# DrQuestion/monica

Measured on AMD Instinct MI355X. Metric: reads/sec classified, higher is better.
Workload: dtype u32/u64 integer; int16 pairs in the alignment kernels (int32 / int8 in the long-call and literal ones); float32 islands: overlap ratio, MAPQ

## Files before the change

monica_amd/csrc/engine.hip:

```cpp
#include <hip/hip_runtime.h>
#include <algorithm>
#include <cmath>
#include <cstdio>
#include <cstring>
#include <cstdlib>
#include <new>
#include <vector>

#include "device.h"
#include <atomic>
#include <thread>

#include "scan.h"

namespace mnc {

void launch_pack(const Batch &B, hipStream_t st);
void launch_sketch(const Batch &B, hipStream_t st);
void launch_partition(const Batch &B, hipStream_t st);
int partition_prepare();
void launch_probe(const Batch &B, hipStream_t st);
void launch_collect(const Batch &B, hipStream_t st);
void launch_expand_sort(const Batch &B, const uint32_t *lists, const ClassSpans &spans, int NM, hipStream_t st);
int expand_sort_prepare(int max_nm);
void launch_backtrack(const Batch &B, const uint32_t *read_list, uint32_t n_list, hipStream_t st);
void launch_bin_reads(const Batch &B, const ChainClasses &C, uint32_t *cls_count, uint32_t *cls_list, hipStream_t st);
void launch_chain_dp_ring(const Batch &B, const uint32_t *lists, const ClassSpans &spans, int stress, hipStream_t st);
void launch_chain_tail(const Batch &B, const uint32_t *lists, const ClassSpans &spans, int NM, hipStream_t st);
size_t chain_tail_lds_bytes(int NM);
int chain_tail_prepare(size_t max_lds);

static const ChainClasses CHAIN_CLASSES = { 22, { 64, 128, 192, 256, 320, 384, 448, 512, 576, 640, 768, 896, 1024, 1280, 1536, 1792, 2048, 2560,
                                                  3072, 4096, 6144, 8192 } };
void launch_regions(const Batch &B, void *regx, uint64_t *k64a, uint64_t *k64b, mnc_hit_t *gated, hipStream_t st);
void launch_regions_post(const Batch &B, mnc_reg_t *work, void *regx, uint64_t *k64a, int32_t *tmp, mnc_hit_t *gated, hipStream_t st);
void launch_dp_gather(const Batch &B, hipStream_t st);
int dp_gather_long_prepare(int lds_anchors);
void launch_dp_gather_long(const Batch &B, const uint32_t *lists, const ClassSpans &spans, int lds_anchors, hipStream_t st);
void launch_dp_round(const Batch &B, int first, hipStream_t st);
void launch_dp_round_end(const Batch &B, hipStream_t st);
int dp_plan_prepare();
void launch_dp_plan(const Batch &B, const int32_t *work_list, unsigned max_work, int wave_form, int state_max, long long p_max, int cig_max,
                    long long big_state, long long big_p, long long big_cig, long long huge_state, long long huge_p, long long huge_cig, hipStream_t st);
size_t dp_align_ws_bytes(long long state_max, long long p_max, long long cig_max);
int dp_align_prepare(int lds_bytes);
int dp_stitch_prepare();
size_t dp_inv_ws_words(int max_gap);
void launch_dp_inv(const Batch &B, const int32_t *work_list, int32_t *next_list, int32_t *ws, int n_wg, hipStream_t st);
size_t dp_stitch_pool_slack(int n_wg);
void launch_dp_align(const Batch &B, uint8_t *ws, int n_wg, long long state_max, long long p_max, long long cig_max,
                     int lds_state, int lds_p, int lds_cig, int big_pass, hipStream_t st, int forms = 3);
void launch_dp_stitch(const Batch &B, const int32_t *work_list, int32_t *next_list, int max_read_len, int n_wg, hipStream_t st);
bool dp_align_long_packed(const Batch &B);
void launch_dp_align_long(const Batch &B, uint8_t *ws_huge, int n_huge, long long st_huge, long long p_huge, long long cig_huge,
                          uint8_t *ws_big, int n_big, long long st_big, long long p_big, long long cig_big,
                          uint8_t *ws_small, int n_small, long long st_small, long long p_small, long long cig_small, hipStream_t st);
size_t dp_fill_p_slot();
size_t dp_fillp_slot();
// ... 48 lines not shown
__global__ __launch_bounds__(PB_N_MAX) void mnc_hist_offsets(const uint32_t *hist_tm, uint32_t n_tiles, uint32_t n_chunks,
                                                             const int64_t *chunk_off_bm, int64_t *q_off)
{
	const uint32_t c = blockIdx.x, b = threadIdx.x, PB_N = blockDim.x;
	const uint32_t t0 = c * HC_TILES, t1 = min(n_tiles, t0 + HC_TILES);
	int64_t run = chunk_off_bm[(size_t)b * n_chunks + c];
	for (uint32_t t = t0; t < t1; ++t) {
		q_off[(size_t)t * PB_N + b] = run;
		run += hist_tm[(size_t)t * PB_N + b];
	}
	if (c == 0 && b == 0) q_off[(size_t)n_tiles * PB_N] = chunk_off_bm[(size_t)PB_N * n_chunks];
}

struct MailItem { const void *src; uint32_t dst_word, n_words; };
constexpr int MAIL_MAX = 8;
struct MailList { MailItem it[MAIL_MAX]; int n; };
__global__ __launch_bounds__(64) void mnc_mail(MailList L, uint32_t *host_box)
{
	for (int k = 0; k < L.n; ++k) {
		const uint32_t *s = static_cast<const uint32_t*>(L.it[k].src);
		for (uint32_t i = threadIdx.x; i < L.it[k].n_words; i += 64) host_box[L.it[k].dst_word + i] = s[i];
	}
	__threadfence_system();
}

struct Buf {
	void *p = nullptr;
	size_t cap = 0;
	int ensure(size_t bytes)
	{
		if (bytes <= cap) return MNC_OK;
		if (p) { (void)hipFree(p); p = nullptr; cap = 0; }
		size_t want = bytes + bytes / 8 + 256;
		hipError_t e = hipMalloc(&p, want);
		if (e != hipSuccess) { p = nullptr; set_error("hipMalloc(%zu) failed: %s", want, hipGetErrorString(e)); return MNC_ERR_NOMEM; }
		cap = want;
		return MNC_OK;
	}
	void release() { if (p) (void)hipFree(p); p = nullptr; cap = 0; }
	template <class T> T *as() const { return reinterpret_cast<T*>(p); }
};

struct SharedWs {
	std::mutex mu;
	int refs = 0;
	Buf fill_p, fill_cig, extp_p, extp_cig, ext_p, lfill_p, lext_p, dp_ws, dp_ws_mid, dp_ws_big, dp_ws_bigfb, dp_ws_huge;
// ... 230 lines not shown
	Buf pf_bases_buf, pf_offsets_buf;
	hipStream_t copy_stream = nullptr;
	hipEvent_t ev_prefetch = nullptr;
	std::mutex pf_mu;
	bool pf_valid = false;
	const uint8_t *pf_bases = nullptr;
	const int64_t *pf_offsets = nullptr;
	uint32_t pf_n = 0;
	int64_t pf_total = 0;
	Buf packed, mz, hits, hist_tm, q_off, qrec, bhits, bhit_cnt;
	size_t q_cap_override = 0;
	Buf ambig, skip, mz_cnt, hit_cnt, rep_len, an_cnt, an_off, n_chain, n_reg, scan_sums, hit_off, best_mlen, hist_sums, hist_offs;
	Buf a, f, p, v, t, u;
	Buf chains_tmp, regs, regx, k64a, k64b, tmp_i32, gated, hits_csr;
	Buf stats, cls_count, cls_list;
	int contract = MNC_CONTRACT_DP;
	Buf ca, ca_cnt, chain_dst, regdp, segs, cig_seg, cig_reg, dp_ctr, work_a, work_b, big_list, huge_list, reg_cnt, regs2;
	SharedWs *ws = nullptr;
	Buf fill1, fill2, fill3, fill_mid, fill_fb, plan_long, extp, mid_list, lfill, lext, bigfb, ext1, ext2, ext3, ext4, gen_list;
	size_t seg_cap_override = 0, cig_cap_override = 0;
	uint32_t *mailbox = nullptr;
	int last_redos = 0;
	long long prev_wide_calls = 0;
	int slot_pad = 2;
	Buf inv_ws;
	int cur_max_read_len = 0;
	int long_reads = 0;
	bool cur_wide = false;
	bool have_merged = false;
	std::vector<int64_t> merged_off;
	std::vector<mnc_hit_t> merged_hits;
	int64_t merged_ctr[24]{};
	Buf ex_off, ex_alns, ex_coff, ex_csoff, ex_mdoff, ex_sums, ex_cigar, ex_cs, ex_md;
	bool ex_valid = false;
	int64_t ex_n_reads = 0, ex_n_aln = 0, ex_n_cig = 0, ex_n_cs = 0, ex_n_md = 0;
	hipEvent_t ev_ex[2]{};
	bool ev_ex_used = false;
	int debug = 0;
	Batch B{};
	bool have_batch = false;
	int64_t last_total_anchors = 0, last_total_hits = -1;
	std::vector<int64_t> h_offsets;
	bool profiling = false;
	hipEvent_t ev[MNC_N_STAGES][2]{};
	bool ev_used[MNC_N_STAGES]{};
	double ms[MNC_N_STAGES]{};
// ... 128 lines not shown
{
	if (n <= e->logf_n) return MNC_OK;
	std::vector<float> lg, lga;
	try { lg.resize((size_t)n), lga.resize((size_t)n); } catch (const std::bad_alloc &) { set_error("out of host memory (MAPQ look-ups)"); return MNC_ERR_NOMEM; }
	for (int i = 0; i < n; ++i) lg[i] = logf((float)i), lga[i] = logf((float)i / e->idx->par.a);
	int rc = e->logf_lut.ensure((size_t)n * 4);
	if (!rc) rc = e->logf_a_lut.ensure((size_t)n * 4);
	if (rc) { e->logf_n = 0; return rc; }
	HIP_TRY(hipMemcpy(e->logf_lut.p, lg.data(), (size_t)n * 4, hipMemcpyHostToDevice));
	HIP_TRY(hipMemcpy(e->logf_a_lut.p, lga.data(), (size_t)n * 4, hipMemcpyHostToDevice));
	e->logf_n = n;
	return MNC_OK;
}

extern "C" int mnc_engine_create(mnc_index *idx, int device, mnc_engine **out)
{
	if (!idx || !out) return MNC_ERR_ARG;
	*out = nullptr;
	if (int rc = check_device(device)) return rc;
	if (idx->par.bw >= GAP_LUT) { set_error("bw too large for the gap look-up"); return MNC_ERR_UNSUPPORTED; }
	mnc_engine *e = new (std::nothrow) mnc_engine;
	if (!e) return MNC_ERR_NOMEM;
	e->idx = idx, e->device = device;
	e->ws = shared_ws(device, +1);
	int rc = index_upload(idx, device, &e->didx);
	if (rc) { mnc_engine_destroy(e); return rc; }
	hipError_t he = hipSetDevice(device);
	int least = 0, greatest = 0;
	if (he == hipSuccess) {
		if (hipDeviceGetStreamPriorityRange(&least, &greatest) != hipSuccess) least = greatest = 0;
		he = hipStreamCreateWithPriority(&e->stream, hipStreamNonBlocking, greatest);
	}
	for (int k = 0; k < mnc_engine::N_SIDE && he == hipSuccess; ++k) {
		he = k < 3 ? hipStreamCreateWithFlags(&e->side[k], hipStreamNonBlocking) : hipStreamCreateWithPriority(&e->side[k], hipStreamNonBlocking, greatest);
		if (he == hipSuccess) he = hipEventCreateWithFlags(&e->ev_join[k], hipEventDisableTiming);
	}
	if (he == hipSuccess) he = hipEventCreateWithFlags(&e->ev_fork, hipEventDisableTiming);
	if (he == hipSuccess) he = hipEventCreateWithFlags(&e->ev_lfill, hipEventDisableTiming);
	if (he == hipSuccess) he = hipStreamCreateWithPriority(&e->copy_stream, hipStreamNonBlocking, least);
	if (he == hipSuccess) he = hipEventCreateWithFlags(&e->ev_prefetch, hipEventDisableTiming);
	if (he == hipSuccess) he = hipHostMalloc((void**)&e->mailbox, 1024, hipHostMallocDefault);
	if (he != hipSuccess) { set_error("stream creation failed: %s", hipGetErrorString(he)); mnc_engine_destroy(e); return MNC_ERR_HIP; }
	for (int s = 0; s < MNC_N_STAGES; ++s) for (int k = 0; k < 2; ++k) (void)hipEventCreate(&e->ev[s][k]);
	std::vector<int32_t> gap(GAP_LUT);
	const float avg_span = (float)idx->k;
	for (int dd = 0; dd < GAP_LUT; ++dd) {
// ... 197 lines not shown
	mark(MNC_STAGE_DP_FILL_T2, 1), mark(MNC_STAGE_DP_FILL_T3, 0);
	launch_dp_fill(B, 128, B.fill_list3, 22, 23, B.fill_fb, 12, B.fill_fb, 12, e->ws->fill_p.as<uint8_t>(), e->ws->fill_cig.as<uint32_t>(), DP_WG_FILL, s0);
	if (!serial && !packed_long && small_batch) long_passes(s0);
	mark(MNC_STAGE_DP_FILL_T3, 1), mark(MNC_STAGE_DP_LFILL, 0);
	if (serial) launch_dp_lfill(B, B.lfill_list, 31, 61, B.fill_fb, 12, e->ws->lfill_p.as<uint8_t>(), DP_WG_LFILL, s0);
	mark(MNC_STAGE_DP_LFILL, 1), mark(MNC_STAGE_DP_EXT, 0);
	for (int i = 7; i >= 0; --i)
		launch_dp_extp(B, 32 << (i >> 1), i & 1, B.extp_list + (int64_t)i * B.seg_cap, 32 + i, 40 + i, e->ws->extp_p.as<uint8_t>(), e->ws->extp_cig.as<uint32_t>(), DP_WG_EXT, s1);
	launch_dp_ext(B, 32, B.ext_list1, 16, 18, B.fill_fb, 12, e->ws->ext_p.as<uint8_t>(), DP_WG_EXT, s1);
	launch_dp_ext(B, 64, B.ext_list2, 17, 19, B.fill_fb, 12, e->ws->ext_p.as<uint8_t>(), DP_WG_EXT, s1);
	launch_dp_ext(B, 128, B.ext_list3, 24, 26, B.fill_fb, 12, e->ws->ext_p.as<uint8_t>(), DP_WG_EXT / 2, s1);
	launch_dp_ext(B, 256, B.ext_list4, 25, 27, B.fill_fb, 12, e->ws->ext_p.as<uint8_t>(), DP_WG_EXT / 4, s1);
	mark(MNC_STAGE_DP_EXT, 1);
	if (serial) {
		launch_dp_lext(B, B.lext_list, 62, 63, B.fill_fb, 12, e->ws->lext_p.as<uint8_t>(), DP_WG_LEXT, s0);
		long_passes(s0);
	}
	launch_dp_align(B, e->ws->dp_ws.as<uint8_t>(), 2 * DP_WG_SMALL, DP_STATE_SMALL, DP_P_SMALL, DP_CIG_SMALL, DP_LDS0_STATE, DP_LDS0_P, DP_LDS0_CIG, 0, s2);
}
static void align_rest(const Batch &B, mnc_engine *e, hipStream_t st)
{
	launch_dp_align(B, e->ws->dp_ws.as<uint8_t>(), DP_WG_SMALL, DP_STATE_SMALL, DP_P_SMALL, DP_CIG_SMALL, DP_LDS_BYTES, 0, 0, 2, st);
	launch_dp_align(B, e->ws->dp_ws_big.as<uint8_t>(), (dp_align_long_packed(B) && !(e->debug & 0x10000)) ? 64 : DP_WG_BIG, DP_STATE_BIG, DP_P_BIG, DP_CIG_BIG, DP_LDS_BYTES, 0, 0, 4, st);
}

static int classify_once(mnc_engine *e, const uint8_t *d_bases, const int64_t *d_offsets,
                         uint32_t n_reads, int64_t total_bases, int min_mapq,
                         int32_t *d_assign, mnc_hit_t *d_best, int32_t *d_nhits, int64_t *d_counts, int *overflowed)
{
	hipStream_t st = e->stream;
	const mnc_index *idx = e->idx;
	*overflowed = 0;
	const size_t nr = (size_t)n_reads, nb = (size_t)total_bases;
	const int pb_bits = e->didx->pb_bits;
	const size_t PB_N = (size_t)1 << pb_bits, PS_TILES = (size_t)(e->cur_wide ? PS_TILES_MIN / 2 : PS_TILES_MIN);
	const size_t n_tiles = (nr + PT_READS - 1) / PT_READS, n_super = (n_tiles + PS_TILES - 1) / PS_TILES;
	size_t q_cap = nb / 3 + 4096;
	if (e->q_cap_override > q_cap) q_cap = e->q_cap_override < nb + 4096 ? e->q_cap_override : nb + 4096;

	int rc = MNC_OK;
#define ENS(buf, bytes) do { if (!rc) rc = e->buf.ensure(bytes); } while (0)
	ENS(packed, (nb / 16 + 4) * 4);
	ENS(mz, (nb + 1) * sizeof(uint2));
	ENS(hits, (nb + 1) * sizeof(HitRec));
	ENS(ambig, (nr + 1) * 4);
	ENS(skip, (nr + 1) * 4);
// ... 43 lines not shown
	B.gap_lut = e->gap_lut.as<int32_t>(), B.logf_lut = e->logf_lut.as<float>(), B.logf_a_lut = e->logf_a_lut.as<float>(), B.logf_n = e->logf_n;
	B.debug_route = (e->debug >> 17 & 15) | ((e->debug >> 22 & 1) << 4) | ((e->debug >> 5 & 1) << 5)
	              | ((e->debug >> 6 & 1) << 6) | ((e->debug >> 7 & 1) << 7)
	              | ((e->debug >> 3 & 1) << 8) | ((e->debug & 1) << 9)
	              | (((unsigned)e->debug >> 31 & 1) << 10);
	B.fill_pred = (e->debug >> 8 & 0xff) ? (e->debug >> 8 & 0xff) : 32;
	B.fill_pred_mid = (e->debug >> 24 & 0x7f) ? (e->debug >> 24 & 0x7f) : 34;
	B.fill_pred_auto = !(e->debug >> 8 & 0xff) && !(e->debug >> 24 & 0x7f) && P.a == 2 && P.b == 4 && P.q == 4 && P.e == 2 &&
	                   P.q2 == 24 && P.e2 == 1 && !getenv("MNC_FILL_PRED_FIXED");
	B.contract = e->contract, B.seq4 = e->didx->seq4, B.seq_off = e->didx->seq_off;
	B.sc_a = P.a, B.sc_b = P.b, B.gap_q = P.q, B.gap_e = P.e, B.gap_q2 = P.q2, B.gap_e2 = P.e2, B.sc_ambi = P.sc_ambi;
	B.zdrop = P.zdrop, B.zdrop_inv = P.zdrop_inv, B.end_bonus = P.end_bonus, B.min_dp_max = P.min_dp_max, B.min_ksw_len = P.min_ksw_len;
	B.max_sw_mat = P.max_sw_mat;
	B.packed = e->packed.as<uint32_t>(), B.ambig = e->ambig.as<uint32_t>(), B.skip = e->skip.as<uint32_t>(), B.mz = e->mz.as<uint2>(), B.hits = e->hits.as<HitRec>();
	B.mz_cnt = e->mz_cnt.as<int32_t>(), B.hit_cnt = e->hit_cnt.as<int32_t>(), B.rep_len = e->rep_len.as<int32_t>();
	B.an_cnt = e->an_cnt.as<int64_t>(), B.an_off = e->an_off.as<int64_t>(), B.n_chain = e->n_chain.as<int32_t>(), B.n_reg = e->n_reg.as<int32_t>(), B.best_mlen = e->best_mlen.as<int32_t>();
	B.n_tiles = (uint32_t)n_tiles, B.n_super = (uint32_t)n_super;
	B.hist_tm = e->hist_tm.as<uint32_t>(), B.q_off = e->q_off.as<int64_t>(), B.qrec = e->qrec.as<uint64_t>();
	B.q_cap = (int64_t)q_cap, B.bhits = e->bhits.as<HitRec>(), B.bhit_cnt = e->bhit_cnt.as<uint32_t>();
	B.overflow = reinterpret_cast<uint32_t*>(e->stats.as<int64_t>() + 8);
	B.assign = d_assign, B.best = d_best, B.nhits = d_nhits ? d_nhits : e->out_nhits.as<int32_t>(), B.counts = d_counts;
	B.stats = e->stats.as<int64_t>();

	HIP_TRY(hipMemsetAsync(B.ambig, 0, (nr + 1) * 4, st));
	HIP_TRY(hipMemsetAsync(B.skip, 0, (nr + 1) * 4, st));
	HIP_TRY(hipMemsetAsync(B.packed + nb / 16, 0, 16, st));
	HIP_TRY(hipMemsetAsync(B.overflow, 0, 8, st));

	{ StageTimer t(e, MNC_STAGE_PACK);   launch_pack(B, st); }
	{ StageTimer t(e, MNC_STAGE_SKETCH); launch_sketch(B, st); }
	{
		StageTimer t(e, MNC_STAGE_PARTITION);
		{
			const uint32_t n_chunks = (uint32_t)((n_tiles + HC_TILES - 1) / HC_TILES);
			uint32_t *sums_bm = e->hist_sums.as<uint32_t>();
			int64_t *off_bm = e->hist_offs.as<int64_t>();
			hipLaunchKernelGGL(mnc_hist_chunk_sums, dim3(n_chunks), dim3((unsigned)PB_N), 0, st, B.hist_tm, (uint32_t)n_tiles, n_chunks, sums_bm);
			exclusive_scan(ScanInPlain<uint32_t>{sums_bm}, (int64_t)n_chunks * PB_N, off_bm, e->scan_sums.as<int64_t>(), st);
			hipLaunchKernelGGL(mnc_hist_offsets, dim3(n_chunks), dim3((unsigned)PB_N), 0, st, B.hist_tm, (uint32_t)n_tiles, n_chunks, off_bm, B.q_off);
		}
		launch_partition(B, st);
	}
	{ StageTimer t(e, MNC_STAGE_PROBE);   launch_probe(B, st); }
	{ StageTimer t(e, MNC_STAGE_COLLECT); launch_collect(B, st); }
	HIP_TRY(hipGetLastError());
	int64_t total_anchors = 0, total_q = 0;
	uint32_t cls_count[MAX_CHAIN_CLASSES + 1] = {0}, overflow = 0;
	{
		StageTimer t(e, MNC_STAGE_SORT);
		exclusive_scan(ScanInPlain<int64_t>{B.an_cnt}, (int64_t)n_reads, B.an_off, e->scan_sums.as<int64_t>(), st);
		HIP_TRY(hipMemsetAsync(e->cls_count.p, 0, (MAX_CHAIN_CLASSES + 1) * 4, st));
		launch_bin_reads(B, CHAIN_CLASSES, e->cls_count.as<uint32_t>(), e->cls_list.as<uint32_t>(), st);
		MailList ml;
		ml.n = 4;
		ml.it[0] = { B.an_off + n_reads, 0, 2 }, ml.it[1] = { B.q_off + n_tiles * PB_N, 2, 2 };
		ml.it[2] = { e->cls_count.p, 4, (uint32_t)(MAX_CHAIN_CLASSES + 1) }, ml.it[3] = { B.overflow, 4 + MAX_CHAIN_CLASSES + 1, 1 };
		hipLaunchKernelGGL(mnc_mail, dim3(1), dim3(64), 0, st, ml, e->mailbox);
		HIP_TRY(hipStreamSynchronize(st));
		memcpy(&total_anchors, e->mailbox, 8), memcpy(&total_q, e->mailbox + 2, 8);
		memcpy(cls_count, e->mailbox + 4, (MAX_CHAIN_CLASSES + 1) * 4);
		overflow = e->mailbox[4 + MAX_CHAIN_CLASSES + 1];
	}
	if (overflow || total_q > (int64_t)q_cap) {
		e->q_cap_override = (size_t)total_q + (size_t)total_q / 8 + 4096;
		*overflowed = 1;
		return MNC_OK;
	}
	if (total_anchors < 0 || total_anchors >= (1LL << 31) * 16) { set_error("anchor count %lld out of range", (long long)total_anchors); return MNC_ERR_UNSUPPORTED; }
	e->last_total_anchors = total_anchors;
	const size_t na = (size_t)total_anchors + 4, ns = (size_t)total_anchors / 3 + 4, nsr = ns + nr * (size_t)e->slot_pad;
	ENS(a, na * sizeof(Anchor));
	ENS(f, na * 4); ENS(p, na * 4); ENS(v, na * 4); ENS(t, na * 4);
	ENS(u, na * 8);
	ENS(chains_tmp, ns * sizeof(ChainRec));
// ... 2 lines not shown
	if (rc) return rc;
#undef ENS
	B.an_cap = (int64_t)na;
	B.slot_pad = e->slot_pad;
	B.a = e->a.as<Anchor>(), B.chains_tmp = e->chains_tmp.as<ChainRec>();
	B.f = e->f.as<int32_t>(), B.p = e->p.as<int32_t>(), B.v = e->v.as<int32_t>(), B.t = e->t.as<int32_t>(), B.u = e->u.as<uint64_t>();
	B.regs = e->regs.as<mnc_reg_t>(), B.tmp_i32 = e->tmp_i32.as<int32_t>();

	auto fork = [&]() -> int {
		HIP_TRY(hipEventRecord(e->ev_fork, st));
		for (int k = 0; k < mnc_engine::N_SIDE; ++k) HIP_TRY(hipStreamWaitEvent(e->side[k], e->ev_fork, 0));
		return MNC_OK;
	};
	auto join = [&]() -> int {
		for (int k = 0; k < mnc_engine::N_SIDE; ++k) {
			HIP_TRY(hipEventRecord(e->ev_join[k], e->side[k]));
			HIP_TRY(hipStreamWaitEvent(st, e->ev_join[k], 0));
		}
		return MNC_OK;
	};
	{
		StageTimer t(e, MNC_STAGE_SORT2);
		const uint32_t *lists = e->cls_list.as<uint32_t>();
		if (int rc = fork()) return rc;
		constexpr int SORT_MERGE = 512;
		int first_big = 0;
		while (first_big < CHAIN_CLASSES.n && CHAIN_CLASSES.nm[first_big] <= SORT_MERGE) ++first_big;
		int k = 0;
		if (first_big > 0) {
			ClassSpans sp;
			sp.n = first_big, sp.stride = (uint32_t)n_reads, sp.start[0] = 0;
			for (int c = 0; c < first_big; ++c) sp.start[c + 1] = sp.start[c] + cls_count[c];
			if (sp.start[sp.n]) launch_expand_sort(B, lists, sp, CHAIN_CLASSES.nm[first_big - 1], e->side[k++ % mnc_engine::N_SIDE]);
		}
		for (int c = first_big; c <= CHAIN_CLASSES.n; ++c) {
			if (cls_count[c] == 0) continue;
			ClassSpans sp;
			sp.n = 1, sp.stride = 0, sp.start[0] = 0, sp.start[1] = cls_count[c];
			launch_expand_sort(B, lists + (size_t)c * n_reads, sp, c < CHAIN_CLASSES.n ? CHAIN_CLASSES.nm[c] : 0,
			                   e->side[k++ % mnc_engine::N_SIDE]);
		}
		if (int rc = join()) return rc;
	}
	{
		StageTimer t(e, MNC_STAGE_CHAIN);
		const uint32_t *lists = e->cls_list.as<uint32_t>();
		ClassSpans spans;
		spans.n = CHAIN_CLASSES.n + 1, spans.stride = (uint32_t)n_reads, spans.start[0] = 0;
		for (int c = 0; c <= CHAIN_CLASSES.n; ++c) spans.start[c + 1] = spans.start[c] + cls_count[c];
		launch_chain_dp_ring(B, lists, spans, (e->debug & 2) != 0, st);
	}
	{
		StageTimer t(e, MNC_STAGE_BACKTRACK);
		const uint32_t *lists = e->cls_list.as<uint32_t>();
		if (int rc = fork()) return rc;
		int k = 0;
		constexpr int merge_to = 384;
		int first_big = 0;
		while (first_big < CHAIN_CLASSES.n && CHAIN_CLASSES.nm[first_big] <= merge_to) ++first_big;
		if (first_big > 0) {
			ClassSpans sp;
			sp.n = first_big, sp.stride = (uint32_t)n_reads, sp.start[0] = 0;
			for (int c = 0; c < first_big; ++c) sp.start[c + 1] = sp.start[c] + cls_count[c];
			if (sp.start[sp.n]) launch_chain_tail(B, lists, sp, CHAIN_CLASSES.nm[first_big - 1], e->side[k++ % mnc_engine::N_SIDE]);
		}
		for (int c = first_big; c < CHAIN_CLASSES.n; ++c) {
			if (cls_count[c] == 0) continue;
			ClassSpans sp;
			sp.n = 1, sp.stride = 0, sp.start[0] = 0, sp.start[1] = cls_count[c];
			launch_chain_tail(B, lists + (size_t)c * n_reads, sp, CHAIN_CLASSES.nm[c], e->side[k++ % mnc_engine::N_SIDE]);
		}
		launch_backtrack(B, lists + (size_t)CHAIN_CLASSES.n * n_reads, cls_count[CHAIN_CLASSES.n], e->side[k % mnc_engine::N_SIDE]);
		if (int rc = join()) return rc;
	}
	if (e->contract == MNC_CONTRACT_DP) {
		size_t seg_cap = na / 6 + 4096, cig_cap = nb / 2 + (1u << 20);
		if (e->seg_cap_override > seg_cap) seg_cap = e->seg_cap_override;
		if (e->cig_cap_override > cig_cap) cig_cap = e->cig_cap_override;
		int rc2 = MNC_OK;
#define ENS2(buf, bytes) do { if (!rc2) rc2 = e->buf.ensure(bytes); } while (0)
#define ENSW(buf, bytes) do { if (!rc2) rc2 = e->ws->buf.ensure(bytes); } while (0)
		std::unique_lock<std::mutex> ws_hold(e->ws->mu);
		ENS2(ca, na * sizeof(Anchor)); ENS2(ca_cnt, (nr + 1) * 4); ENS2(chain_dst, ns * 4); ENS2(regdp, nsr * sizeof(RegDP));
		ENS2(inv_ws, dp_inv_ws_words(B.max_gap) * 4 * DP_WG_INV);
		const size_t cig_reg_cap = cig_cap + dp_stitch_pool_slack(DP_WG_STITCH);
		ENS2(segs, seg_cap * sizeof(Seg)); ENS2(cig_seg, cig_cap * 4); ENS2(cig_reg, cig_reg_cap * 4);
		ENS2(work_a, nsr * 4); ENS2(work_b, nsr * 4); ENS2(big_list, seg_cap * 4); ENS2(reg_cnt, (nr + 1) * 4); ENS2(regs2, nsr * sizeof(mnc_reg_t));
		const size_t ws_small = dp_align_ws_bytes(DP_STATE_SMALL, DP_P_SMALL, DP_CIG_SMALL), ws_big = dp_align_ws_bytes(DP_STATE_BIG, DP_P_BIG, DP_CIG_BIG), ws_huge = dp_align_ws_bytes(DP_STATE_HUGE, DP_P_HUGE, DP_CIG_HUGE);
		ENSW(dp_ws, ws_small * DP_WG_SMALL * 2); ENSW(dp_ws_big, ws_big * DP_WG_BIG); ENSW(dp_ws_bigfb, ws_big * DP_WG_BIGFB); ENSW(dp_ws_huge, ws_huge * DP_WG_HUGE); ENS2(huge_list, seg_cap * 4); ENSW(dp_ws_mid, ws_small * DP_WG_MID); ENS2(mid_list, seg_cap * 4); ENS2(lfill, seg_cap * 4); ENSW(lfill_p, dp_lfill_p_slot() * DP_WG_LFILL); ENS2(lext, seg_cap * 4); ENS2(bigfb, seg_cap * 4); ENSW(lext_p, dp_lext_p_slot() * DP_WG_LEXT);
		ENS2(plan_long, (nr * 4 + 1024) * 4);
		ENS2(fill1, seg_cap * 4); ENS2(fill2, seg_cap * 4); ENS2(fill3, seg_cap * 4); ENS2(fill_mid, seg_cap * 4); ENS2(fill_fb, seg_cap * 4); ENSW(fill_p, dp_fillp_slot() * DP_WG_FILL); ENSW(fill_cig, dp_fillp_cig_slot() * DP_WG_FILL); ENS2(extp, seg_cap * 4 * 8); ENSW(extp_p, dp_extp_slot() * DP_WG_EXT); ENSW(extp_cig, dp_extp_cig_slot() * DP_WG_EXT); ENS2(ext1, seg_cap * 4); ENS2(ext2, seg_cap * 4); ENS2(ext3, seg_cap * 4); ENS2(ext4, seg_cap * 4); ENS2(gen_list, seg_cap * 4); ENSW(ext_p, dp_fill_p_slot() * DP_WG_EXT);
#undef ENS2
		if (rc2) return rc2;
		B.ca = e->ca.as<Anchor>(), B.ca_cnt = e->ca_cnt.as<int32_t>(), B.chain_dst = e->chain_dst.as<int32_t>(), B.regdp = e->regdp.as<RegDP>();
		B.segs = e->segs.as<Seg>(), B.seg_cap = (int64_t)seg_cap, B.cig_seg = e->cig_seg.as<uint32_t>(), B.cig_reg = e->cig_reg.as<uint32_t>();
		B.cig_seg_cap = (int64_t)cig_cap, B.cig_reg_cap = (int64_t)cig_reg_cap, B.dp_ctr = e->dp_ctr.as<unsigned long long>();
		B.big_list = e->big_list.as<int32_t>(), B.huge_list = e->huge_list.as<int32_t>(), B.reg_cnt = e->reg_cnt.as<int32_t>();
		B.plan_long_list = e->plan_long.as<int32_t>(), B.plan_long_cap = (long long)(nr * 4 + 1024);
		B.fill_list1 = e->fill1.as<int32_t>(), B.fill_list2 = e->fill2.as<int32_t>(), B.fill_list3 = e->fill3.as<int32_t>(), B.fill_list_mid = e->fill_mid.as<int32_t>(), B.fill_fb = e->fill_fb.as<int32_t>();
		B.ext_list1 = e->ext1.as<int32_t>(), B.ext_list2 = e->ext2.as<int32_t>(), B.ext_list3 = e->ext3.as<int32_t>(), B.ext_list4 = e->ext4.as<int32_t>(), B.gen_list = e->gen_list.as<int32_t>(), B.extp_list = e->extp.as<int32_t>(), B.mid_list = e->mid_list.as<int32_t>(), B.lfill_list = e->lfill.as<int32_t>(), B.lext_list = e->lext.as<int32_t>(), B.bigfb_list = e->bigfb.as<int32_t>();
		B.lds0_state = DP_LDS0_STATE, B.lds0_p = DP_LDS0_P, B.lds0_cig = DP_LDS0_CIG;
		int32_t *lists[2] = { e->work_a.as<int32_t>(), e->work_b.as<int32_t>() };
		B.next_list = lists[0];
		HIP_TRY(hipMemsetAsync(e->dp_ctr.p, 0, 64 * 8, st));
		{ StageTimer t(e, MNC_STAGE_REGIONS);   launch_regions(B, e->regx.p, e->k64a.as<uint64_t>(), e->k64b.as<uint64_t>(), e->gated.as<mnc_hit_t>(), st); }
		{
			StageTimer t(e, MNC_STAGE_DP_PLAN);
			launch_dp_gather(B, st);
			int c0 = 0;
			while (c0 < CHAIN_CLASSES.n && CHAIN_CLASSES.nm[c0] <= 1024) ++c0;
			ClassSpans sp;
			sp.n = CHAIN_CLASSES.n + 1 - c0, sp.stride = (uint32_t)n_reads, sp.start[0] = 0;
			for (int c = c0; c <= CHAIN_CLASSES.n; ++c) sp.start[c - c0 + 1] = sp.start[c - c0] + cls_count[c];
			launch_dp_gather_long(B, e->cls_list.as<uint32_t>() + (size_t)c0 * n_reads, sp, CHAIN_CLASSES.nm[CHAIN_CLASSES.n - 1], st);
		}
		unsigned max_work = (unsigned)nsr;
		const int long_reads = (e->debug & 0x10) ? 2 : (e->debug & 0x800000) ? 0 : n_reads <= 4096 ? 2
		                     : (e->cur_max_read_len <= 0 || e->cur_max_read_len > 6144) ? 1 : 0;
		for (int round = 0;; ++round) {
			const int32_t *work = lists[round & 1];
			int32_t *next = lists[(round + 1) & 1];
			B.next_list = next;
			launch_dp_round(B, round == 0, st);
			if (round == 0) {
				{ StageTimer t(e, MNC_STAGE_DP_PLAN);   launch_dp_plan(B, work, max_work, long_reads, (int)DP_STATE_SMALL, DP_P_SMALL, (int)DP_CIG_SMALL, DP_STATE_BIG, DP_P_BIG, DP_CIG_BIG, DP_STATE_HUGE, DP_P_HUGE, DP_CIG_HUGE, st); }
				{
					StageTimer t(e, MNC_STAGE_DP_FILL);
					if (int rcf = fork()) return rcf;
					if (e->debug & 0x10000) align_round(B, e, e->side[0], e->side[0], e->side[0], e->side[0], e->side[0]);
					else align_round(B, e, e->side[0], e->side[1], st, e->side[2], e->side[3]);
					if (int rcj = join()) return rcj;
				}
				{
					StageTimer t(e, MNC_STAGE_DP_ALIGN);
					align_rest(B, e, st);
				}
				{ StageTimer t(e, MNC_STAGE_DP_STITCH); launch_dp_stitch(B, work, next, (e->debug & 0x200000) ? 0 : e->cur_max_read_len > 0 ? e->cur_max_read_len : 8192, DP_WG_STITCH, st); }
			} else {
				launch_dp_plan(B, work, max_work, long_reads, (int)DP_STATE_SMALL, DP_P_SMALL, (int)DP_CIG_SMALL, DP_STATE_BIG, DP_P_BIG, DP_CIG_BIG, DP_STATE_HUGE, DP_P_HUGE, DP_CIG_HUGE, st);
				if (int rcf = fork()) return rcf;
				if (e->debug & 0x10000) align_round(B, e, e->side[0], e->side[0], e->side[0], e->side[0], e->side[0]);
				else align_round(B, e, e->side[0], e->side[1], st, e->side[2], e->side[3]);
				if (int rcj = join()) return rcj;
				align_rest(B, e, st);
				launch_dp_stitch(B, work, next, (e->debug & 0x200000) ? 0 : e->cur_max_read_len > 0 ? e->cur_max_read_len : 8192, DP_WG_STITCH, st);
				launch_dp_inv(B, work, next, e->inv_ws.as<int32_t>(), (int)std::min<unsigned>(DP_WG_INV, max_work), st);
			}
			launch_dp_round_end(B, st);
			unsigned long long ctr[6] = {0};
			{
				MailList ml;
				ml.n = 3;
				ml.it[0] = { e->dp_ctr.p, 0, 12 };
				ml.it[1] = { e->dp_ctr.as<unsigned long long>() + 6, 12, 2 }, ml.it[2] = { e->dp_ctr.as<unsigned long long>() + 58, 14, 2 };
				hipLaunchKernelGGL(mnc_mail, dim3(1), dim3(64), 0, st, ml, e->mailbox);
				HIP_TRY(hipStreamSynchronize(st));
				memcpy(ctr, e->mailbox, sizeof(ctr));
				if (round == 0 && n_reads >= 4096) {
					unsigned long long big = 0, huge = 0;
					memcpy(&big, e->mailbox + 12, 8), memcpy(&huge, e->mailbox + 14, 8);
					e->prev_wide_calls = (long long)(big + huge);
				}
			}
			if (ctr[4] != 0) {
				if (ctr[4] >= 9) { set_error("a gap between two seeds is too large for the alignment workspace"); return MNC_ERR_UNSUPPORTED; }
				if (ctr[4] == 5) {
					e->slot_pad = e->slot_pad * 4;
					*overflowed = 2;
					return MNC_OK;
				}
				e->seg_cap_override = na + 2 * ns + 1024;
				e->cig_cap_override = cig_cap * 4;
				*overflowed = 2;
				return MNC_OK;
			}
			if (ctr[5] == 0) break;
			if (round > 256) { set_error("base-level alignment does not settle"); return MNC_ERR_HIP; }
			max_work = (unsigned)ctr[5];
		}
		{ StageTimer t(e, MNC_STAGE_DP_POST); launch_regions_post(B, e->regs2.as<mnc_reg_t>(), e->regx.p, e->k64a.as<uint64_t>(), e->tmp_i32.as<int32_t>(), e->gated.as<mnc_hit_t>(), st); }
	} else {
		StageTimer t(e, MNC_STAGE_REGIONS);
		launch_regions(B, e->regx.p, e->k64a.as<uint64_t>(), e->k64b.as<uint64_t>(), e->gated.as<mnc_hit_t>(), st);
	}
	HIP_TRY(hipGetLastError());
	e->have_batch = true;
	return MNC_OK;
}

extern "C" int mnc_classify_device(mnc_engine *e, const uint8_t *d_bases, const int64_t *d_offsets,
                                   uint32_t n_reads, int64_t total_bases, int max_read_len, int min_mapq,
                                   int32_t *d_assign, mnc_hit_t *d_best, int32_t *d_nhits, int64_t *d_counts)
{
	if (!e || !d_offsets || !d_assign || (total_bases > 0 && !d_bases) || total_bases < 0) return MNC_ERR_ARG;
	if (((uintptr_t)d_bases & 15u) != 0) { set_error("d_bases must be 16-byte aligned"); return MNC_ERR_ARG; }
	const bool wide = e->long_reads && max_read_len >= (1 << QPOS_BITS);
	if (max_read_len < 0 || (wide ? max_read_len > MNC_MAX_READ_LEN_WIDE : max_read_len >= (1 << QPOS_BITS))) {
		set_error(e->long_reads ? "reads beyond 2^24 - 1 bases are not supported" : "reads of 2^20 bases or more are not supported (mnc_engine_set_long_reads)");
		return MNC_ERR_UNSUPPORTED;
	}
	if (n_reads > (1u << 20)) { set_error("at most 2^20 reads per batch (query records hold a 20-bit read ordinal)"); return MNC_ERR_UNSUPPORTED; }
	if (wide && n_reads > (uint32_t)WIDE_MAX_READS) { set_error("at most 2^16 reads in a call with reads of 2^20 bases or more (wide query records hold a 16-bit read ordinal)"); return MNC_ERR_UNSUPPORTED; }
	if (total_bases >= (1LL << 40)) return MNC_ERR_UNSUPPORTED;
// ... 545 lines not shown
```

monica_amd/csrc/k_post.hip:

```cpp
#include "device.h"

namespace mnc {

__device__ __forceinline__ uint64_t mix64(uint64_t key)
{
	key = ~key + (key << 21);
	key = key ^ key >> 24;
	key = (key + (key << 3)) + (key << 8);
	key = key ^ key >> 14;
	key = (key + (key << 2)) + (key << 4);
	key = key ^ key >> 28;
	key = key + (key << 31);
	return key;
}

__device__ __forceinline__ uint32_t wang32(uint32_t key)
{
	key += ~(key << 15);
	key ^=  (key >> 10);
	key +=  (key << 3);
	key ^=  (key >> 6);
	key += ~(key << 11);
	key ^=  (key >> 16);
	return key;
// ... 393 lines not shown
			for (int i = 0; i < n_regs; ++i) total += rg[i].cnt;
			B.ca_cnt[rd] = total;
			if (n_regs > 0) {
				const unsigned long long w0 = atomicAdd(&B.dp_ctr[5], (unsigned long long)n_regs);
				for (int i = 0; i < n_regs; ++i) {
					RegDP d;
					memset(&d, 0, sizeof(d));
					d.read = (int32_t)rd, d.order = i << 8, d.state = 1;
					B.regdp[slot + i] = d;
					B.next_list[w0 + i] = (int32_t)(slot + i);
				}
			}
		}
	} else if (dp) B.ca_cnt[rd] = 0;
	if (dp) { B.reg_cnt[rd] = n_regs; return; }
	B.n_reg[rd] = n_regs;
	B.assign[rd] = assign;
	if (B.best) B.best[rd] = best;
	B.nhits[rd] = nhits;
	B.best_mlen[rd] = best.mlen;
}

__global__ __launch_bounds__(64) void mnc_regions_post(Batch B, mnc_reg_t *work_all, RegX *regx_all, uint64_t *k64a_all,
                                                       int32_t *tmp_all, mnc_hit_t *gated_all)
{
	const uint32_t rd = blockIdx.x * blockDim.x + threadIdx.x;
	if (rd >= B.n_reads) return;
	int32_t assign = MNC_UNMAPPED, nhits = 0;
	mnc_hit_t best;
	best.rid = best.mapq = best.nm = best.mlen = 0;
	const int n0 = B.reg_cnt[rd];
	int n_regs = 0;
	if (n0 > 0) {
		const int64_t slot = reg_slot(B, rd);
		mnc_reg_t *src = B.regs + slot, *r = work_all + slot;
		RegX *ex = regx_all + slot;
		uint64_t *ka = k64a_all + slot;
		int32_t *w = tmp_all + slot * 4, *tmp = w + n0;
		mnc_hit_t *gated = gated_all + slot;
		for (int i = 0; i < n0; ++i) w[i] = i;
		for (int i = 1; i < n0; ++i) {
			const int c = w[i], oc = B.regdp[slot + c].order;
			int j = i - 1;
			while (j >= 0 && B.regdp[slot + w[j]].order > oc) { w[j + 1] = w[j]; --j; }
			w[j + 1] = c;
		}
		int k = 0;
		for (int i = 0; i < n0; ++i) {
			const mnc_reg_t x = src[w[i]];
			bool flt = !(x.flags & REG_INV) && x.cnt < B.min_cnt;
// ... 23 lines not shown
			}
			for (int i = 0; i < n_regs; ++i) src[i] = r[tmp[i]], B.regdp[slot + i].cig_off = (int64_t)ex[tmp[i]].x0;
			for (int i = 0; i < n_regs; ++i) { r[i] = src[i]; RegX e; e.x0 = (uint64_t)B.regdp[slot + i].cig_off, e.y0 = 0, e.x1 = (uint64_t)(uint32_t)src[i].n_cigar, e.y1 = 0; ex[i] = e; }
		}
		set_parent(B, n_regs, r, ka, w);
		n_regs = select_sub(B, n_regs, r, ex, tmp);
		set_mapq(B, rd, n_regs, r);
		gate_and_decide(B, n_regs, r, gated, assign, best, nhits);
		for (int i = 0; i < n_regs; ++i) src[i] = r[i], B.regdp[slot + i].cig_off = (int64_t)ex[i].x0, B.regdp[slot + i].n_cigar = r[i].n_cigar;
	}
	if (B.skip[rd]) {
		assign = MNC_SKIPPED, nhits = 0;
		memset(&best, 0, sizeof(best));
	}
	B.n_reg[rd] = n_regs;
	B.assign[rd] = assign;
	if (B.best) B.best[rd] = best;
	B.nhits[rd] = nhits;
	B.best_mlen[rd] = best.mlen;
}

constexpr int CT_THREADS = 256, CT_READS = 4096, CT_LDS_BINS = 3 * 1024;

__global__ __launch_bounds__(CT_THREADS) void mnc_count_taxa(Batch B)
{
	__shared__ unsigned long long s_bins[CT_LDS_BINS];
	const int n_bins = B.n_genomes * 3;
	const bool in_lds = n_bins <= CT_LDS_BINS;
	if (in_lds) {
		for (int k = threadIdx.x; k < n_bins; k += CT_THREADS) s_bins[k] = 0;
		__syncthreads();
	}
	unsigned long long *bins = in_lds ? s_bins : (unsigned long long*)B.counts;
	const uint32_t lo = blockIdx.x * CT_READS;
	const uint32_t hi = min(B.n_reads, lo + CT_READS);
	for (uint32_t rd = lo + threadIdx.x; rd < hi; rd += CT_THREADS) {
		const int a = B.assign[rd];
		if (a < 0) continue;
		const int g = B.contig_genome[a];
		atomicAdd(&bins[g * 3 + 0], 1ULL);
		atomicAdd(&bins[g * 3 + 1], (unsigned long long)(B.offsets[rd + 1] - B.offsets[rd]));
		atomicAdd(&bins[g * 3 + 2], (unsigned long long)B.best_mlen[rd]);
	}
	if (in_lds) {
		__syncthreads();
		for (int k = threadIdx.x; k < n_bins; k += CT_THREADS)
			if (s_bins[k]) atomicAdd((unsigned long long*)&B.counts[k], s_bins[k]);
	}
}

__global__ __launch_bounds__(256) void mnc_gather_hits(Batch B, const mnc_hit_t *gated_all,
                                                       const int64_t *hit_off, mnc_hit_t *out)
{
	const uint32_t rd = blockIdx.x * blockDim.x + threadIdx.x;
	if (rd >= B.n_reads) return;
	const int n = B.nhits[rd];
	if (n == 0) return;
	const mnc_hit_t *src = gated_all + reg_slot(B, rd);
	mnc_hit_t *dst = out + hit_off[rd];
	for (int i = 0; i < n; ++i) dst[i] = src[i];
}

void launch_regions(const Batch &B, void *regx, uint64_t *k64a, uint64_t *k64b, mnc_hit_t *gated, hipStream_t st)
{
	if (B.n_reads == 0) return;
	hipLaunchKernelGGL(mnc_regions_decide, dim3((B.n_reads + 63) / 64), dim3(64), 0, st, B,
	                   reinterpret_cast<RegX*>(regx), k64a, k64b, gated);
	if (B.counts && B.contract != MNC_CONTRACT_DP)
		hipLaunchKernelGGL(mnc_count_taxa, dim3((B.n_reads + CT_READS - 1) / CT_READS), dim3(CT_THREADS), 0, st, B);
}

void launch_regions_post(const Batch &B, mnc_reg_t *work, void *regx, uint64_t *k64a, int32_t *tmp, mnc_hit_t *gated, hipStream_t st)
{
	if (B.n_reads == 0) return;
	hipLaunchKernelGGL(mnc_regions_post, dim3((B.n_reads + 63) / 64), dim3(64), 0, st, B, work,
	                   reinterpret_cast<RegX*>(regx), k64a, tmp, gated);
	if (B.counts) hipLaunchKernelGGL(mnc_count_taxa, dim3((B.n_reads + CT_READS - 1) / CT_READS), dim3(CT_THREADS), 0, st, B);
}

void launch_gather_hits(const Batch &B, const mnc_hit_t *gated, const int64_t *hit_off, mnc_hit_t *out, hipStream_t st)
{
	if (B.n_reads == 0) return;
	hipLaunchKernelGGL(mnc_gather_hits, dim3((B.n_reads + 255) / 256), dim3(256), 0, st, B, gated, hit_off, out);
}

}
```

Measured before the change: 2.875 million.

## Fuse batch clears into one kernel, gate side-stream fork, speculatively queue post stage

Replaces the per-batch hipMemsetAsync calls (ambig, skip, packed tail, overflow, class counts, DP counters) with a single clearing kernel. It forks onto side streams for the sort and backtrack stages only when the work outside the largest class exceeds a threshold, and otherwise launches everything on the main stream. It also queues the regions-post and count-taxa kernels before the first host sync, gated on device counters so they exit early if more DP rounds are needed. The aim is fewer API calls, fewer cross-stream event waits and less idle time after the host sync, at the cost of more complex control flow and possibly lost overlap for small batches. The old behaviour is kept behind the MNC_HOST_WAITS environment variable.

```diff
diff --git a/monica_amd/csrc/engine.hip b/monica_amd/csrc/engine.hip
--- a/monica_amd/csrc/engine.hip
+++ b/monica_amd/csrc/engine.hip
@@ -33,7 +33,7 @@
 static const ChainClasses CHAIN_CLASSES = { 22, { 64, 128, 192, 256, 320, 384, 448, 512, 576, 640, 768, 896, 1024, 1280, 1536, 1792, 2048, 2560,
                                                   3072, 4096, 6144, 8192 } };
 void launch_regions(const Batch &B, void *regx, uint64_t *k64a, uint64_t *k64b, mnc_hit_t *gated, hipStream_t st);
-void launch_regions_post(const Batch &B, mnc_reg_t *work, void *regx, uint64_t *k64a, int32_t *tmp, mnc_hit_t *gated, hipStream_t st);
+void launch_regions_post(const Batch &B, mnc_reg_t *work, void *regx, uint64_t *k64a, int32_t *tmp, mnc_hit_t *gated, const unsigned long long *gate, hipStream_t st);
 void launch_dp_gather(const Batch &B, hipStream_t st);
 int dp_gather_long_prepare(int lds_anchors);
 void launch_dp_gather_long(const Batch &B, const uint32_t *lists, const ClassSpans &spans, int lds_anchors, hipStream_t st);
@@ -128,6 +128,20 @@
 		for (uint32_t i = threadIdx.x; i < L.it[k].n_words; i += 64) host_box[L.it[k].dst_word + i] = s[i];
 	}
 	__threadfence_system();
+}
+
+static_assert(MAX_CHAIN_CLASSES + 1 <= 256, "mnc_clear_batch clears the class counts with one workgroup");
+__global__ __launch_bounds__(256) void mnc_clear_batch(uint32_t *ambig, uint32_t *skip, uint32_t n_words, uint32_t *packed_tail,
+                                                       uint32_t *overflow, uint32_t *cls_count, unsigned long long *dp_ctr)
+{
+	const uint32_t stride = gridDim.x * blockDim.x;
+	for (uint32_t i = blockIdx.x * blockDim.x + threadIdx.x; i < n_words; i += stride) ambig[i] = 0, skip[i] = 0;
+	if (blockIdx.x == 0) {
+		if (threadIdx.x < 4) packed_tail[threadIdx.x] = 0;
+		if (threadIdx.x < 2) overflow[threadIdx.x] = 0;
+		if (threadIdx.x <= MAX_CHAIN_CLASSES) cls_count[threadIdx.x] = 0;
+		if (dp_ctr && threadIdx.x < 64) dp_ctr[threadIdx.x] = 0;
+	}
 }
 
 struct Buf {
@@ -404,6 +418,7 @@
 	uint32_t *mailbox = nullptr;
 	int last_redos = 0;
 	long long prev_wide_calls = 0;
+	bool host_waits = false;
 	int slot_pad = 2;
 	Buf inv_ws;
 	int cur_max_read_len = 0;
@@ -578,6 +593,10 @@
 	mnc_engine *e = new (std::nothrow) mnc_engine;
 	if (!e) return MNC_ERR_NOMEM;
 	e->idx = idx, e->device = device;
+	{
+		const char *hw = getenv("MNC_HOST_WAITS");
+		e->host_waits = hw && atoi(hw) != 0;
+	}
 	e->ws = shared_ws(device, +1);
 	int rc = index_upload(idx, device, &e->didx);
 	if (rc) { mnc_engine_destroy(e); return rc; }
@@ -821,6 +840,19 @@
 {
 	launch_dp_align(B, e->ws->dp_ws.as<uint8_t>(), DP_WG_SMALL, DP_STATE_SMALL, DP_P_SMALL, DP_CIG_SMALL, DP_LDS_BYTES, 0, 0, 2, st);
 	launch_dp_align(B, e->ws->dp_ws_big.as<uint8_t>(), (dp_align_long_packed(B) && !(e->debug & 0x10000)) ? 64 : DP_WG_BIG, DP_STATE_BIG, DP_P_BIG, DP_CIG_BIG, DP_LDS_BYTES, 0, 0, 4, st);
+}
+
+constexpr uint64_t BESIDE_MIN = 10'000'000;
+static uint64_t slots_beside_largest(const uint32_t *cls_count, int first_big, bool with_last)
+{
+	uint64_t all = 0, largest = 0, small = 0;
+	for (int c = 0; c < first_big; ++c) small += (uint64_t)cls_count[c] * CHAIN_CLASSES.nm[c];
+	all = largest = small;
+	for (int c = first_big; c < CHAIN_CLASSES.n + (with_last ? 1 : 0); ++c) {
+		const uint64_t w = (uint64_t)cls_count[c] * CHAIN_CLASSES.nm[std::min(c, CHAIN_CLASSES.n - 1)];
+		all += w, largest = std::max(largest, w);
+	}
+	return all - largest;
 }
 
 static int classify_once(mnc_engine *e, const uint8_t *d_bases, const int64_t *d_offsets,
@@ -910,10 +942,17 @@
 	B.assign = d_assign, B.best = d_best, B.nhits = d_nhits ? d_nhits : e->out_nhits.as<int32_t>(), B.counts = d_counts;
 	B.stats = e->stats.as<int64_t>();
 
-	HIP_TRY(hipMemsetAsync(B.ambig, 0, (nr + 1) * 4, st));
-	HIP_TRY(hipMemsetAsync(B.skip, 0, (nr + 1) * 4, st));
-	HIP_TRY(hipMemsetAsync(B.packed + nb / 16, 0, 16, st));
-	HIP_TRY(hipMemsetAsync(B.overflow, 0, 8, st));
+	const bool host_waits = e->host_waits;
+	if (host_waits) {
+		HIP_TRY(hipMemsetAsync(B.ambig, 0, (nr + 1) * 4, st));
+		HIP_TRY(hipMemsetAsync(B.skip, 0, (nr + 1) * 4, st));
+		HIP_TRY(hipMemsetAsync(B.packed + nb / 16, 0, 16, st));
+		HIP_TRY(hipMemsetAsync(B.overflow, 0, 8, st));
+	} else {
+		const unsigned blocks = (unsigned)std::min<size_t>((nr + 1 + 255) / 256, 1024);
+		hipLaunchKernelGGL(mnc_clear_batch, dim3(blocks), dim3(256), 0, st, B.ambig, B.skip, (uint32_t)(nr + 1), B.packed + nb / 16, B.overflow,
+		                   e->cls_count.as<uint32_t>(), e->contract == MNC_CONTRACT_DP ? e->dp_ctr.as<unsigned long long>() : nullptr);
+	}
 
 	{ StageTimer t(e, MNC_STAGE_PACK);   launch_pack(B, st); }
 	{ StageTimer t(e, MNC_STAGE_SKETCH); launch_sketch(B, st); }
@@ -937,7 +976,7 @@
 	{
 		StageTimer t(e, MNC_STAGE_SORT);
 		exclusive_scan(ScanInPlain<int64_t>{B.an_cnt}, (int64_t)n_reads, B.an_off, e->scan_sums.as<int64_t>(), st);
-		HIP_TRY(hipMemsetAsync(e->cls_count.p, 0, (MAX_CHAIN_CLASSES + 1) * 4, st));
+		if (host_waits) HIP_TRY(hipMemsetAsync(e->cls_count.p, 0, (MAX_CHAIN_CLASSES + 1) * 4, st));
 		launch_bin_reads(B, CHAIN_CLASSES, e->cls_count.as<uint32_t>(), e->cls_list.as<uint32_t>(), st);
 		MailList ml;
 		ml.n = 4;
@@ -986,25 +1025,28 @@
 	{
 		StageTimer t(e, MNC_STAGE_SORT2);
 		const uint32_t *lists = e->cls_list.as<uint32_t>();
-		if (int rc = fork()) return rc;
 		constexpr int SORT_MERGE = 512;
 		int first_big = 0;
 		while (first_big < CHAIN_CLASSES.n && CHAIN_CLASSES.nm[first_big] <= SORT_MERGE) ++first_big;
+		uint32_t n_small = 0;
+		for (int c = 0; c < first_big; ++c) n_small += cls_count[c];
+		const bool beside = host_waits || slots_beside_largest(cls_count, first_big, true) > BESIDE_MIN;
+		if (beside) if (int rc = fork()) return rc;
 		int k = 0;
-		if (first_big > 0) {
+		auto where = [&]() { return beside ? e->side[k++ % mnc_engine::N_SIDE] : st; };
+		if (n_small) {
 			ClassSpans sp;
 			sp.n = first_big, sp.stride = (uint32_t)n_reads, sp.start[0] = 0;
 			for (int c = 0; c < first_big; ++c) sp.start[c + 1] = sp.start[c] + cls_count[c];
-			if (sp.start[sp.n]) launch_expand_sort(B, lists, sp, CHAIN_CLASSES.nm[first_big - 1], e->side[k++ % mnc_engine::N_SIDE]);
+			launch_expand_sort(B, lists, sp, CHAIN_CLASSES.nm[first_big - 1], where());
 		}
 		for (int c = first_big; c <= CHAIN_CLASSES.n; ++c) {
 			if (cls_count[c] == 0) continue;
 			ClassSpans sp;
 			sp.n = 1, sp.stride = 0, sp.start[0] = 0, sp.start[1] = cls_count[c];
-			launch_expand_sort(B, lists + (size_t)c * n_reads, sp, c < CHAIN_CLASSES.n ? CHAIN_CLASSES.nm[c] : 0,
-			                   e->side[k++ % mnc_engine::N_SIDE]);
-		}
-		if (int rc = join()) return rc;
+			launch_expand_sort(B, lists + (size_t)c * n_reads, sp, c < CHAIN_CLASSES.n ? CHAIN_CLASSES.nm[c] : 0, where());
+		}
+		if (beside) if (int rc = join()) return rc;
 	}
 	{
 		StageTimer t(e, MNC_STAGE_CHAIN);
@@ -1017,25 +1059,29 @@
 	{
 		StageTimer t(e, MNC_STAGE_BACKTRACK);
 		const uint32_t *lists = e->cls_list.as<uint32_t>();
-		if (int rc = fork()) return rc;
-		int k = 0;
 		constexpr int merge_to = 384;
 		int first_big = 0;
 		while (first_big < CHAIN_CLASSES.n && CHAIN_CLASSES.nm[first_big] <= merge_to) ++first_big;
-		if (first_big > 0) {
+		uint32_t n_small = 0;
+		for (int c = 0; c < first_big; ++c) n_small += cls_count[c];
+		const bool beside = host_waits || slots_beside_largest(cls_count, first_big, true) > BESIDE_MIN;
+		if (beside) if (int rc = fork()) return rc;
+		int k = 0;
+		auto where = [&]() { return beside ? e->side[k++ % mnc_engine::N_SIDE] : st; };
+		if (n_small) {
 			ClassSpans sp;
 			sp.n = first_big, sp.stride = (uint32_t)n_reads, sp.start[0] = 0;
 			for (int c = 0; c < first_big; ++c) sp.start[c + 1] = sp.start[c] + cls_count[c];
-			if (sp.start[sp.n]) launch_chain_tail(B, lists, sp, CHAIN_CLASSES.nm[first_big - 1], e->side[k++ % mnc_engine::N_SIDE]);
+			launch_chain_tail(B, lists, sp, CHAIN_CLASSES.nm[first_big - 1], where());
 		}
 		for (int c = first_big; c < CHAIN_CLASSES.n; ++c) {
 			if (cls_count[c] == 0) continue;
 			ClassSpans sp;
 			sp.n = 1, sp.stride = 0, sp.start[0] = 0, sp.start[1] = cls_count[c];
-			launch_chain_tail(B, lists + (size_t)c * n_reads, sp, CHAIN_CLASSES.nm[c], e->side[k++ % mnc_engine::N_SIDE]);
-		}
-		launch_backtrack(B, lists + (size_t)CHAIN_CLASSES.n * n_reads, cls_count[CHAIN_CLASSES.n], e->side[k % mnc_engine::N_SIDE]);
-		if (int rc = join()) return rc;
+			launch_chain_tail(B, lists + (size_t)c * n_reads, sp, CHAIN_CLASSES.nm[c], where());
+		}
+		launch_backtrack(B, lists + (size_t)CHAIN_CLASSES.n * n_reads, cls_count[CHAIN_CLASSES.n], where());
+		if (beside) if (int rc = join()) return rc;
 	}
 	if (e->contract == MNC_CONTRACT_DP) {
 		size_t seg_cap = na / 6 + 4096, cig_cap = nb / 2 + (1u << 20);
@@ -1066,7 +1112,7 @@
 		B.lds0_state = DP_LDS0_STATE, B.lds0_p = DP_LDS0_P, B.lds0_cig = DP_LDS0_CIG;
 		int32_t *lists[2] = { e->work_a.as<int32_t>(), e->work_b.as<int32_t>() };
 		B.next_list = lists[0];
-		HIP_TRY(hipMemsetAsync(e->dp_ctr.p, 0, 64 * 8, st));
+		if (host_waits) HIP_TRY(hipMemsetAsync(e->dp_ctr.p, 0, 64 * 8, st));
 		{ StageTimer t(e, MNC_STAGE_REGIONS);   launch_regions(B, e->regx.p, e->k64a.as<uint64_t>(), e->k64b.as<uint64_t>(), e->gated.as<mnc_hit_t>(), st); }
 		{
 			StageTimer t(e, MNC_STAGE_DP_PLAN);
@@ -1081,6 +1127,7 @@
 		unsigned max_work = (unsigned)nsr;
 		const int long_reads = (e->debug & 0x10) ? 2 : (e->debug & 0x800000) ? 0 : n_reads <= 4096 ? 2
 		                     : (e->cur_max_read_len <= 0 || e->cur_max_read_len > 6144) ? 1 : 0;
+		bool post_queued = false;
 		for (int round = 0;; ++round) {
 			const int32_t *work = lists[round & 1];
 			int32_t *next = lists[(round + 1) & 1];
@@ -1118,6 +1165,11 @@
 				ml.it[0] = { e->dp_ctr.p, 0, 12 };
 				ml.it[1] = { e->dp_ctr.as<unsigned long long>() + 6, 12, 2 }, ml.it[2] = { e->dp_ctr.as<unsigned long long>() + 58, 14, 2 };
 				hipLaunchKernelGGL(mnc_mail, dim3(1), dim3(64), 0, st, ml, e->mailbox);
+				if (round == 0 && !host_waits) {
+					StageTimer t(e, MNC_STAGE_DP_POST);
+					launch_regions_post(B, e->regs2.as<mnc_reg_t>(), e->regx.p, e->k64a.as<uint64_t>(), e->tmp_i32.as<int32_t>(), e->gated.as<mnc_hit_t>(), B.dp_ctr, st);
+					post_queued = true;
+				}
 				HIP_TRY(hipStreamSynchronize(st));
 				memcpy(ctr, e->mailbox, sizeof(ctr));
 				if (round == 0 && n_reads >= 4096) {
@@ -1139,10 +1191,11 @@
 				return MNC_OK;
 			}
 			if (ctr[5] == 0) break;
+			post_queued = false;
 			if (round > 256) { set_error("base-level alignment does not settle"); return MNC_ERR_HIP; }
 			max_work = (unsigned)ctr[5];
 		}
-		{ StageTimer t(e, MNC_STAGE_DP_POST); launch_regions_post(B, e->regs2.as<mnc_reg_t>(), e->regx.p, e->k64a.as<uint64_t>(), e->tmp_i32.as<int32_t>(), e->gated.as<mnc_hit_t>(), st); }
+		if (!post_queued) { StageTimer t(e, MNC_STAGE_DP_POST); launch_regions_post(B, e->regs2.as<mnc_reg_t>(), e->regx.p, e->k64a.as<uint64_t>(), e->tmp_i32.as<int32_t>(), e->gated.as<mnc_hit_t>(), nullptr, st); }
 	} else {
 		StageTimer t(e, MNC_STAGE_REGIONS);
 		launch_regions(B, e->regx.p, e->k64a.as<uint64_t>(), e->k64b.as<uint64_t>(), e->gated.as<mnc_hit_t>(), st);
diff --git a/monica_amd/csrc/k_post.hip b/monica_amd/csrc/k_post.hip
--- a/monica_amd/csrc/k_post.hip
+++ b/monica_amd/csrc/k_post.hip
@@ -439,10 +439,11 @@
 }
 
 __global__ __launch_bounds__(64) void mnc_regions_post(Batch B, mnc_reg_t *work_all, RegX *regx_all, uint64_t *k64a_all,
-                                                       int32_t *tmp_all, mnc_hit_t *gated_all)
+                                                       int32_t *tmp_all, mnc_hit_t *gated_all, const unsigned long long *gate)
 {
 	const uint32_t rd = blockIdx.x * blockDim.x + threadIdx.x;
 	if (rd >= B.n_reads) return;
+	if (gate && (gate[4] | gate[5]) != 0) return;
 	int32_t assign = MNC_UNMAPPED, nhits = 0;
 	mnc_hit_t best;
 	best.rid = best.mapq = best.nm = best.mlen = 0;
@@ -512,8 +513,9 @@
 
 constexpr int CT_THREADS = 256, CT_READS = 4096, CT_LDS_BINS = 3 * 1024;
 
-__global__ __launch_bounds__(CT_THREADS) void mnc_count_taxa(Batch B)
-{
+__global__ __launch_bounds__(CT_THREADS) void mnc_count_taxa(Batch B, const unsigned long long *gate)
+{
+	if (gate && (gate[4] | gate[5]) != 0) return;
 	__shared__ unsigned long long s_bins[CT_LDS_BINS];
 	const int n_bins = B.n_genomes * 3;
 	const bool in_lds = n_bins <= CT_LDS_BINS;
@@ -557,15 +559,15 @@
 	hipLaunchKernelGGL(mnc_regions_decide, dim3((B.n_reads + 63) / 64), dim3(64), 0, st, B,
 	                   reinterpret_cast<RegX*>(regx), k64a, k64b, gated);
 	if (B.counts && B.contract != MNC_CONTRACT_DP)
-		hipLaunchKernelGGL(mnc_count_taxa, dim3((B.n_reads + CT_READS - 1) / CT_READS), dim3(CT_THREADS), 0, st, B);
-}
-
-void launch_regions_post(const Batch &B, mnc_reg_t *work, void *regx, uint64_t *k64a, int32_t *tmp, mnc_hit_t *gated, hipStream_t st)
+		hipLaunchKernelGGL(mnc_count_taxa, dim3((B.n_reads + CT_READS - 1) / CT_READS), dim3(CT_THREADS), 0, st, B, (const unsigned long long*)nullptr);
+}
+
+void launch_regions_post(const Batch &B, mnc_reg_t *work, void *regx, uint64_t *k64a, int32_t *tmp, mnc_hit_t *gated, const unsigned long long *gate, hipStream_t st)
 {
 	if (B.n_reads == 0) return;
 	hipLaunchKernelGGL(mnc_regions_post, dim3((B.n_reads + 63) / 64), dim3(64), 0, st, B, work,
-	                   reinterpret_cast<RegX*>(regx), k64a, tmp, gated);
-	if (B.counts) hipLaunchKernelGGL(mnc_count_taxa, dim3((B.n_reads + CT_READS - 1) / CT_READS), dim3(CT_THREADS), 0, st, B);
+	                   reinterpret_cast<RegX*>(regx), k64a, tmp, gated, gate);
+	if (B.counts) hipLaunchKernelGGL(mnc_count_taxa, dim3((B.n_reads + CT_READS - 1) / CT_READS), dim3(CT_THREADS), 0, st, B, gate);
 }
 
 void launch_gather_hits(const Batch &B, const mnc_hit_t *gated, const int64_t *hit_off, mnc_hit_t *out, hipStream_t st)
```

New measurement: 2.878 million, median of 2. No clear change (+0.1%).
